# bryanboateng/animating-gaussian-splats

Measured on AMD Instinct MI355X. Metric: Msplats/sec fwd+bwd @1080p (1M gauss), higher is better.
Workload: dtype f32; 1 GPU; C3: 1000000 Gaussians, SH3, 1920x1080, 27-camera rig, 5 view(s)/GPU/step, fwd+bwd; gaussians=1000000, image=1920x1080, sh_degree=3, parallelism=camera-dp1, streams_per_gpu=3, submission=one host thread per stream, means2D=one fresh zero leaf per render (shared.py:38-41)

## Files before the change

animating-gaussian-splats_amd/csrc/gsr_forward.hip:

```cpp
#include "gsr_common.h"
#include "gsr_internal.h"

#include <algorithm>
#include <type_traits>

namespace gsr {

#ifdef GSR_TRACE
__device__ uint64_t *g_trace_fwd;
#ifdef GSR_TRACE
__device__ inline uint64_t trace_fwd_work(uint64_t batches, uint64_t walk, uint64_t evals) {
    return (batches << 40) | ((walk < 0xFFFFFull ? walk : 0xFFFFFull) << 20) | (evals < 0xFFFFFull ? evals : 0xFFFFFull);
}
#endif
__device__ uint64_t *g_trace_emit;
#define GSR_EMIT_STAMP(k)                                                                        \
    do {                                                                                         \
        if (g_trace_emit && threadIdx.x == 0)                                                    \
            g_trace_emit[4 * blockIdx.x + (k)] = __builtin_amdgcn_s_memrealtime();               \
    } while (0)
#else
#define GSR_EMIT_STAMP(k) do {} while (0)
#endif

// ... 225 lines not shown
            ranges[tl] = cnt ? make_uint2(ex, ex + cnt) : make_uint2(0, 0);
            tile_cursor[tl] = ex;
            seg_off[tl] = ex_s + is - sb;
            if (cnt > (uint32_t)kSortCap) {
                sort_lists[T - 1 - atomicAdd(&ctr[3], 1u)] = (uint32_t)tl;
                atomicMax(&ctr[4], cnt);
            } else if (cnt > (uint32_t)kFwdSortCap) {
                sort_lists[atomicAdd(&ctr[2], 1u)] = (uint32_t)tl;
            }
        }
    }
    drain_vmem();
    __builtin_amdgcn_fence(__ATOMIC_RELEASE, "workgroup");
    __syncthreads();
    if (threadIdx.x == 0) s_last = atomicAdd(&ctr[1], 1u) == gridDim.x - 1 ? 1u : 0u;
    __syncthreads();
    if (!s_last) return;
    const uint64_t fin = __hip_atomic_load(&look[gridDim.x - 1], __ATOMIC_RELAXED, __HIP_MEMORY_SCOPE_AGENT);
    const uint32_t K = (uint32_t)fin, n_seg = (uint32_t)(fin >> 32) & 0x3FFFFFFFu;
    {
        constexpr int kPer = kOrderBuckets / (kColW * kColG);
        uint32_t h[kPer], hs = 0;
#pragma unroll
        for (int i = 0; i < kPer; ++i) {
            h[i] = __hip_atomic_load(&lpt[threadIdx.x * kPer + i], __ATOMIC_RELAXED, __HIP_MEMORY_SCOPE_AGENT);
            hs += h[i];
        }
        uint32_t tt;
        uint32_t e = block_excl_scan_u32(hs, s_red, &tt);
#pragma unroll
        for (int i = 0; i < kPer; ++i) {
            lpt[threadIdx.x * kPer + i] = e;
            e += h[i];
        }
    }
    {
        const uint32_t bs = (int)threadIdx.x < NB ? block_sums[threadIdx.x] : 0u;
        uint32_t btot;
        const uint32_t bex = block_excl_scan_u32(bs, s_red, &btot);
        if ((int)threadIdx.x < NB) block_off[threadIdx.x] = bex;
    }
    if (threadIdx.x == 0) {
        const uint32_t n_mid = __hip_atomic_load(&ctr[2], __ATOMIC_RELAXED, __HIP_MEMORY_SCOPE_AGENT);
        const uint32_t n_long = __hip_atomic_load(&ctr[3], __ATOMIC_RELAXED, __HIP_MEMORY_SCOPE_AGENT);
        const uint32_t max_long = __hip_atomic_load(&ctr[4], __ATOMIC_RELAXED, __HIP_MEMORY_SCOPE_AGENT);
        seg_off[T] = n_seg;
        meta[0] = K;
        meta[1] = (cap && K <= cap && n_long == 0u) ? 1u : 0u;
        meta[2] = n_mid;
        if (host_words) {
            __hip_atomic_store(host_words + 1, n_mid, __ATOMIC_RELAXED, __HIP_MEMORY_SCOPE_SYSTEM);
            __hip_atomic_store(host_words + 2, n_long, __ATOMIC_RELAXED, __HIP_MEMORY_SCOPE_SYSTEM);
            __hip_atomic_store(host_words + 3, max_long, __ATOMIC_RELAXED, __HIP_MEMORY_SCOPE_SYSTEM);
            __hip_atomic_store(host_words, K, __ATOMIC_RELEASE, __HIP_MEMORY_SCOPE_SYSTEM);
        }
    }
}

__global__ __launch_bounds__(1024) void k_bin_scan(int T, int NB, const uint32_t *__restrict__ tile_count,
                                                   uint2 *__restrict__ ranges,
                                                   uint32_t *__restrict__ tile_cursor,
                                                   const uint32_t *__restrict__ block_sums,
                                                   uint32_t *__restrict__ block_off,
                                                   uint32_t *__restrict__ meta,
                                                   uint32_t *host_words,
                                                   uint32_t *__restrict__ tile_order,
                                                   uint32_t *__restrict__ sort_lists,
                                                   uint32_t *__restrict__ seg_off, uint32_t cap, int ks) {
    __shared__ uint32_t s_red[16];
    __shared__ uint32_t s_hist[kOrderBuckets];
    __shared__ uint32_t s_cls[3];
    if (threadIdx.x < 3) s_cls[threadIdx.x] = 0;
    uint32_t carry = 0;
    for (int base = 0; base < T; base += blockDim.x) {
        const int t = base + threadIdx.x;
        const uint32_t c = t < T ? tile_count[t] : 0;
        uint32_t tot;
        const uint32_t ex = block_excl_scan_u32(c, s_red, &tot) + carry;
        if (t < T) {
            ranges[t] = c ? make_uint2(ex, ex + c) : make_uint2(0, 0);
            tile_cursor[t] = ex;
        }
        carry += tot;
    }
    uint32_t carry3 = 0;
    for (int base = 0; base < T; base += blockDim.x) {
        const int t = base + threadIdx.x;
        const uint32_t nb = t < T ? seg_bounds(tile_count[t], ks) : 0;
        uint32_t tot;
        const uint32_t ex = block_excl_scan_u32(nb, s_red, &tot) + carry3;
        if (t < T) seg_off[t] = ex;
        carry3 += tot;
    }
    if (threadIdx.x == 0) seg_off[T] = carry3;
    uint32_t carry2 = 0;
    for (int base = 0; base < NB; base += blockDim.x) {
        const int b = base + threadIdx.x;
        const uint32_t c = b < NB ? block_sums[b] : 0;
        uint32_t tot;
        const uint32_t ex = block_excl_scan_u32(c, s_red, &tot) + carry2;
        if (b < NB) block_off[b] = ex;
        carry2 += tot;
    }
    __syncthreads();
    for (int t = threadIdx.x; t < T; t += blockDim.x) {
        const uint32_t n = tile_count[t];
        if (n == 0) continue;
        if (n > (uint32_t)kSortCap) {
            sort_lists[T - 1 - atomicAdd(&s_cls[1], 1u)] = (uint32_t)t;
            atomicMax(&s_cls[2], n);
        } else if (n > (uint32_t)kFwdSortCap) {
            sort_lists[atomicAdd(&s_cls[0], 1u)] = (uint32_t)t;
        }
    }
    lds_barrier();
    if (threadIdx.x == 0) {
        meta[0] = carry;
        meta[1] = (cap && carry <= cap && s_cls[1] == 0u) ? 1u : 0u;
        meta[2] = s_cls[0];
        if (host_words) {
            for (int c = 0; c < 3; ++c)
                __hip_atomic_store(host_words + 1 + c, s_cls[c], __ATOMIC_RELAXED, __HIP_MEMORY_SCOPE_SYSTEM);
            __hip_atomic_store(host_words, carry, __ATOMIC_RELEASE, __HIP_MEMORY_SCOPE_SYSTEM);
        }
    }
    lpt_order(T, [&](int t) { return tile_count[t]; }, tile_order, s_hist, s_red);
}

template <bool USE_LDS>
__global__ __launch_bounds__(kBinThreads) void k_bin_emit(int P, int CH, int T, int gx,
                                                  const uint2 *__restrict__ rects,
                                                  const uint32_t *__restrict__ tiles,
                                                  const float *__restrict__ depth,
                                                  const uint32_t *__restrict__ block_off,
                                                  uint32_t *__restrict__ tile_cursor,
                                                  uint32_t *__restrict__ goff,
                                                  uint4 *__restrict__ pairs, uint32_t K,
                                                  const uint32_t *__restrict__ chunk_off,
                                                  const uint32_t *__restrict__ spec_ok,
                                                  const uint32_t *__restrict__ tile_count,
                                                  const uint32_t *__restrict__ tile_rank,
                                                  const uint32_t *__restrict__ lpt_off,
                                                  uint32_t *__restrict__ tile_order) {
    extern __shared__ __attribute__((aligned(16))) uint32_t s_cur[];
    __shared__ uint32_t s_red[16];
    if (spec_ok && *spec_ok == 0u) return;
    const int b = blockIdx.x;
    const int g0 = b * CH, g1 = min(P, g0 + CH);
    if (tile_rank) {
        const int per = div_up(T, (int)gridDim.x), t1 = min(T, (b + 1) * per);
        for (int t = b * per + (int)threadIdx.x; t < t1; t += blockDim.x)
            tile_order[lpt_off[lpt_bucket(tile_count[t])] + tile_rank[t]] = (uint32_t)t;
    }
    GSR_EMIT_STAMP(0);
    if (USE_LDS) {
        const uint32_t *row = chunk_off + (size_t)b * T;
        for (int t = threadIdx.x; t < T; t += blockDim.x) s_cur[t] = tile_cursor[t] + row[t];
        __syncthreads();
        GSR_EMIT_STAMP(1);
        GSR_EMIT_STAMP(2);
    }
    uint32_t carry = block_off[b];
    for (int base = g0; base < g1; base += blockDim.x) {
        const int g = base + threadIdx.x;
        const uint32_t n = g < g1 ? tiles[g] : 0;
        uint32_t tot;
        const uint32_t ex = block_excl_scan_u32(n, s_red, &tot) + carry;
        carry += tot;
        if (g < g1) {
            goff[g] = ex;
            if (n) {
                const uint2 r = rects[g];
                const int x0 = r.x & 0xFFFF, y0 = r.x >> 16, x1 = r.y & 0xFFFF, y1 = r.y >> 16;
                const uint32_t dbits = __float_as_uint(depth[g]);
                uint32_t e = ex;
                for (int y = y0; y < y1; ++y)
                    for (int x = x0; x < x1; ++x, ++e) {
                        const int t = y * gx + x;
                        const uint32_t pos = USE_LDS ? atomicAdd(&s_cur[t], 1u) : atomicAdd(&tile_cursor[t], 1u);
                        pairs[pos] = make_uint4((uint32_t)g, dbits, e, 0u);
                    }
            }
        }
    }
    if (b == gridDim.x - 1 && threadIdx.x == 0) goff[P] = spec_ok ? spec_ok[-1] : K;
#ifdef GSR_TRACE
    __syncthreads();
    GSR_EMIT_STAMP(3);
#endif
}


template <int D>
__device__ inline uint32_t lane_xor(uint32_t x) {
    if constexpr (D == 1) return (uint32_t)__builtin_amdgcn_mov_dpp((int)x, 0xB1, 0xF, 0xF, false);
    else if constexpr (D == 2) return (uint32_t)__builtin_amdgcn_mov_dpp((int)x, 0x4E, 0xF, 0xF, false);
    else if constexpr (D == 4) {
        const int m = __builtin_amdgcn_mov_dpp((int)x, 0x141, 0xF, 0xF, false);
        return (uint32_t)__builtin_amdgcn_mov_dpp(m, 0x1B, 0xF, 0xF, false);
    } else if constexpr (D == 8) return (uint32_t)__builtin_amdgcn_mov_dpp((int)x, 0x128, 0xF, 0xF, false);
    else if constexpr (D == 16) {
        auto r = __builtin_amdgcn_permlane16_swap(x, x, false, false);
        return (threadIdx.x & 16) ? r[0] : r[1];
    } else {
        auto r = __builtin_amdgcn_permlane32_swap(x, x, false, false);
        return (threadIdx.x & 32) ? r[0] : r[1];
    }
}

template <int R, int D>
__device__ inline void bitonic_xlane(uint64_t (&k)[R], uint32_t (&v)[R], bool take_min) {
#pragma unroll
    for (int r = 0; r < R; ++r) {
        const uint32_t plo = lane_xor<D>((uint32_t)k[r]), phi = lane_xor<D>((uint32_t)(k[r] >> 32));
        const uint32_t pv = lane_xor<D>(v[r]);
        const uint64_t pk = ((uint64_t)phi << 32) | plo;
        const bool mine = (k[r] < pk) == take_min;
        k[r] = mine ? k[r] : pk;
        v[r] = mine ? v[r] : pv;
    }
}

template <int R, int J>
__device__ inline void wave_merge_stages(uint64_t (&k)[R], uint32_t (&v)[R], int lane, uint32_t gbase, uint32_t KK) {
    if constexpr (J > 0) {
        if constexpr (J < R) {
#pragma unroll
            for (int r = 0; r < R; ++r) {
                if (r & J) continue;
                const int r2 = r | J;
                const bool asc = ((gbase + lane * R + r) & KK) == 0;
                if ((k[r] > k[r2]) == asc) {
                    const uint64_t t = k[r]; k[r] = k[r2]; k[r2] = t;
                    const uint32_t u = v[r]; v[r] = v[r2]; v[r2] = u;
                }
            }
        } else {
            constexpr int D = J / R;
            const bool asc = ((gbase + lane * R) & KK) == 0;
            const bool take_min = ((lane & D) == 0) == asc;
            bitonic_xlane<R, D>(k, v, take_min);
        }
        wave_merge_stages<R, J / 2>(k, v, lane, gbase, KK);
    }
}

template <int R, int KK>
__device__ inline void wave_sort_stages(uint64_t (&k)[R], uint32_t (&v)[R], int lane, uint32_t gbase) {
    if constexpr (KK <= 64 * R) {
        wave_merge_stages<R, KK / 2>(k, v, lane, gbase, KK);
        wave_sort_stages<R, 2 * KK>(k, v, lane, gbase);
    }
}

__device__ inline uint32_t sort_slot(uint32_t i) { return i + (i >> 4); }
constexpr int sort_slots(int n) { return n + n / 16; }

template <int R>
__device__ inline void block_xchg_stage(uint64_t (&k)[R], uint32_t (&v)[R], uint32_t ibase, int kk, int j,
                                        uint64_t *s_key, uint32_t *s_val) {
    const uint32_t sb = sort_slot(ibase), qb = sort_slot(ibase ^ (uint32_t)j);
#pragma unroll
    for (int r = 0; r < R; ++r) { s_key[sb + r] = k[r]; s_val[sb + r] = v[r]; }
    __syncthreads();
#pragma unroll
    for (int r = 0; r < R; ++r) {
        const uint32_t i = ibase + r;
        const uint64_t pk = s_key[qb + r];
        const uint32_t pv = s_val[qb + r];
        const bool take_min = ((i & j) == 0) == ((i & kk) == 0);
        const bool mine = (k[r] < pk) == take_min;
        k[r] = mine ? k[r] : pk;
        v[r] = mine ? v[r] : pv;
    }
    __syncthreads();
}

template <int R, int NW>
__device__ inline void block_sort_tile(int n, uint32_t start, const uint4 *__restrict__ pairs, uint64_t *s_key,
                                       uint32_t *s_val) {
    constexpr int SEG = 64 * R;
    const int lane = threadIdx.x & 63, w = threadIdx.x >> 6;
    const uint32_t gbase = (uint32_t)(w * SEG), ibase = gbase + lane * R;
    uint64_t k[R];
    uint32_t v[R];
#pragma unroll
    for (int r = 0; r < R; ++r) {
        const int i = (int)ibase + r;
        const uint4 q = i < n ? pairs[start + i] : make_uint4(~0u, ~0u, 0u, 0u);
        k[r] = pair_key(q);
        v[r] = q.z;
    }
    wave_sort_stages<R, 2>(k, v, lane, gbase);
    for (uint32_t kk = 2 * SEG; kk <= (uint32_t)(NW * SEG); kk <<= 1) {
        for (uint32_t j = kk >> 1; j >= (uint32_t)SEG; j >>= 1) block_xchg_stage<R>(k, v, ibase, kk, j, s_key, s_val);
        wave_merge_stages<R, SEG / 2>(k, v, lane, gbase, kk);
    }
    const uint32_t sb = sort_slot(ibase);
#pragma unroll
    for (int r = 0; r < R; ++r) { s_key[sb + r] = k[r]; s_val[sb + r] = v[r]; }
    __syncthreads();
}

__global__ __launch_bounds__(512) void k_tile_sort(int gx, const uint32_t *__restrict__ tiles,
                                                    const uint2 *__restrict__ ranges,
                                                    uint4 *__restrict__ pairs,
                                                    uint32_t *__restrict__ point_list,
                                                    uint32_t *__restrict__ slot_emit, uint32_t nlist,
                                                    const uint32_t *__restrict__ spec_ok) {
    __shared__ uint64_t s_keys[sort_slots(kSortCap)];
    __shared__ uint32_t s_vals[sort_slots(kSortCap)];
    if (spec_ok) {
        if (*spec_ok == 0u) return;
        nlist = spec_ok[1];
    }
    static_assert(kSortCap == 8 * 64 * 8, "k_tile_sort: 8 waves x 64 lanes x 8 keys");
    for (uint32_t li = blockIdx.x; li < nlist; li += gridDim.x) {
        const int tile = (int)tiles[li];
        const uint2 rg = ranges[tile];
        const int n = (int)(rg.y - rg.x);
        if (n <= 4 * 64 * 8) block_sort_tile<4, 8>(n, rg.x, pairs, s_keys, s_vals);
        else block_sort_tile<8, 8>(n, rg.x, pairs, s_keys, s_vals);
        for (int i = threadIdx.x; i < n; i += blockDim.x) {
            const uint32_t sl = sort_slot((uint32_t)i);
            point_list[rg.x + i] = (uint32_t)s_keys[sl];
            slot_emit[rg.x + i] = s_vals[sl];
        }
        __syncthreads();
    }
}

__device__ inline uint4 key_record(uint64_t k, uint32_t emit) {
    return make_uint4((uint32_t)k, (uint32_t)(k >> 32), emit, 0u);
}

__global__ __launch_bounds__(512) void k_chunk_sort(int T, const uint32_t *__restrict__ lists,
                                                     const uint2 *__restrict__ ranges, uint4 *__restrict__ pairs) {
    __shared__ uint64_t s_keys[sort_slots(kSortCap)];
    __shared__ uint32_t s_vals[sort_slots(kSortCap)];
    const int tile = (int)lists[T - 1 - (int)blockIdx.y];
    const uint2 rg = ranges[tile];
    const int n = (int)(rg.y - rg.x);
    const int c0 = (int)blockIdx.x * kSortCap;
    if (c0 >= n) return;
    const int m = min(kSortCap, n - c0);
    block_sort_tile<8, 8>(m, rg.x + c0, pairs, s_keys, s_vals);
    for (int i = threadIdx.x; i < m; i += blockDim.x) {
        const uint32_t sl = sort_slot((uint32_t)i);
        pairs[rg.x + c0 + i] = key_record(s_keys[sl], s_vals[sl]);
    }
}

__device__ inline uint32_t merge_split(const uint4 *__restrict__ a, uint32_t la, const uint4 *__restrict__ b,
                                       uint32_t lb, uint32_t d) {
    const int lane = threadIdx.x & 63;
    uint32_t lo = d > lb ? d - lb : 0u, hi = min(d, la);
    while (lo < hi) {
        const uint32_t span = hi - lo, step = (span + 63) / 64;
        const uint32_t x = lo + (uint32_t)lane * step;
        const bool p = x < hi && pair_key(a[x]) < pair_key(b[d - 1 - x]);
        const uint32_t c = (uint32_t)__popcll(__ballot(p));
        const uint32_t nlo = c ? lo + (c - 1) * step + 1 : lo;
        const uint32_t nhi = min(hi, lo + c * step);
        lo = nlo;
        hi = max(nlo, nhi);
    }
    return lo;
}

__global__ __launch_bounds__(512) void k_merge_pass(int T, const uint32_t *__restrict__ lists,
                                                     const uint2 *__restrict__ ranges, uint32_t L,
                                                     const uint4 *__restrict__ src, uint4 *__restrict__ dst,
                                                     int final_pass, uint32_t *__restrict__ point_list,
                                                     uint32_t *__restrict__ slot_emit) {
    __shared__ uint64_t s_ka[kSortCap], s_kb[kSortCap];
    __shared__ uint32_t s_va[kSortCap], s_vb[kSortCap];
    __shared__ uint32_t s_split[2];
    const int tile = (int)lists[T - 1 - (int)blockIdx.y];
    const uint2 rg = ranges[tile];
    const uint32_t n = rg.y - rg.x;
    const uint32_t o0 = blockIdx.x * (uint32_t)kSortCap;
    if (o0 >= n) return;
    const uint32_t pb = o0 / (2 * L) * (2 * L);
    const uint32_t la = min(L, n - pb), lb = n - pb > L ? min(L, n - pb - L) : 0u;
    const uint4 *a = src + rg.x + pb, *b = a + la;
    const uint32_t d0 = o0 - pb, d1 = min(d0 + (uint32_t)kSortCap, la + lb);
    const int wv = threadIdx.x >> 6;
    if (wv < 2) {
        const uint32_t sp = merge_split(a, la, b, lb, wv == 0 ? d0 : d1);
        if ((threadIdx.x & 63) == 0) s_split[wv] = sp;
    }
    __syncthreads();
    const uint32_t i0 = s_split[0], i1 = s_split[1], j0 = d0 - i0, j1 = d1 - i1;
    const uint32_t na = i1 - i0, nb = j1 - j0;
    for (uint32_t i = threadIdx.x; i < na; i += blockDim.x) { const uint4 q = a[i0 + i]; s_ka[i] = pair_key(q); s_va[i] = q.z; }
    for (uint32_t i = threadIdx.x; i < nb; i += blockDim.x) { const uint4 q = b[j0 + i]; s_kb[i] = pair_key(q); s_vb[i] = q.z; }
    __syncthreads();
    constexpr uint32_t kPer = kSortCap / 512;
    const uint32_t dl = threadIdx.x * kPer;
    if (dl >= na + nb) return;
    uint32_t lo = dl > nb ? dl - nb : 0u, hi = min(dl, na);
    while (lo < hi) {
        const uint32_t mid = (lo + hi) >> 1;
        if (s_ka[mid] < s_kb[dl - 1 - mid]) lo = mid + 1; else hi = mid;
    }
    uint32_t ia = lo, ib = dl - lo;
    const uint32_t e = min(dl + kPer, na + nb);
    for (uint32_t o = dl; o < e; ++o) {
        const bool take_a = ib >= nb || (ia < na && s_ka[ia] < s_kb[ib]);
        const uint64_t k = take_a ? s_ka[ia] : s_kb[ib];
        const uint32_t v = take_a ? s_va[ia] : s_vb[ib];
        ia += take_a; ib += !take_a;
        const size_t slot = (size_t)rg.x + pb + d0 + o;
        if (final_pass) { point_list[slot] = (uint32_t)k; slot_emit[slot] = v; }
        else dst[slot] = key_record(k, v);
    }
}

__device__ inline void gate_wait(const uint32_t *gate, uint32_t seq, uint32_t *err, uint64_t timeout) {
    const uint64_t t0 = __builtin_amdgcn_s_memrealtime();
    while ((int32_t)(__hip_atomic_load(gate, __ATOMIC_ACQUIRE, __HIP_MEMORY_SCOPE_SYSTEM) - seq) < 0) {
        __builtin_amdgcn_s_sleep(100);
        if (__builtin_amdgcn_s_memrealtime() - t0 > timeout) {
            if (threadIdx.x == 0 &&
                (int32_t)(__hip_atomic_load(gate, __ATOMIC_ACQUIRE, __HIP_MEMORY_SCOPE_SYSTEM) - seq) < 0)
                __hip_atomic_store(err, seq, __ATOMIC_RELAXED, __HIP_MEMORY_SCOPE_SYSTEM);
            return;
        }
    }
}

#ifndef GSR_TSAT_THREADS
#define GSR_TSAT_THREADS 64
#endif
constexpr int kTSatThreads = GSR_TSAT_THREADS;
__device__ inline bool tsat_flagged(float T, uint32_t last) { return T < kTSat * (1.0f + t_window(last)); }
struct TSatRec { float4 r0, r1, r3; };
__device__ inline TSatRec tsat_load(const float4 *__restrict__ rec, uint32_t g, bool v) {
    TSatRec t;
    const float4 z = make_float4(0.f, 0.f, 0.f, 0.f);
    const float4 *r = rec + (size_t)kRecF4 * g;
    t.r0 = v ? r[0] : z; t.r1 = v ? r[1] : z; t.r3 = v ? r[3] : z;
    return t;
}
__device__ inline void tsat_chain(int nf, const uint32_t *__restrict__ plist, float pfx, float pfy,
                                  const float4 *__restrict__ rec, uint32_t *s_rc, float *s_q, float *s_a,
                                  uint32_t *s_pos, float &T, uint32_t &nex, float4 &E) {
    constexpr int NT = kTSatThreads, NW = NT / 64;
    const int t = threadIdx.x, lane = t & 63, wv = t >> 6;
    float Tc = 0.f;
    bool stopped = false;
    uint32_t g_next = t < nf ? plist[t] : 0u;
    TSatRec cur = tsat_load(rec, g_next, t < nf);
    g_next = NT + t < nf ? plist[NT + t] : 0u;
    for (int base = 0; base < nf; base += NT) {
        const int e = base + t;
        const TSatRec r = cur;
        cur = tsat_load(rec, g_next, e + NT < nf);
        g_next = e + 2 * NT < nf ? plist[e + 2 * NT] : 0u;
        bool take = false;
        float al = 0.f;
        if (e < nf) {
            const Blend eb = blend_eval<true>(r.r0, r.r1, pfx, pfy);
            if (eb.p2 <= 0.0f && eb.alpha >= kNearLo) {
                const ExactBlend x = exact_blend(r.r0.x, r.r0.y, r.r3, r.r1.y, pfx, pfy);
                take = eb.alpha >= kNearHi || (x.power <= 0.0f && x.alpha >= 1.0f / 255.0f);
                al = x.alpha;
            }
        }
        const uint64_t m = __ballot(take);
        if (lane == 0) s_rc[wv] = (uint32_t)__builtin_popcountll(m);
        __syncthreads();
        uint32_t off = 0, nc = 0;
#pragma unroll
        for (int w = 0; w < NW; ++w) {
            off += w < wv ? s_rc[w] : 0u;
            nc += s_rc[w];
        }
        if (take) {
            const uint32_t rk = off + __builtin_amdgcn_mbcnt_hi((uint32_t)(m >> 32), __builtin_amdgcn_mbcnt_lo((uint32_t)m, 0u));
            s_q[rk] = 1.0f - al;
            s_a[rk] = al;
            s_pos[rk] = (uint32_t)e;
        }
        if (t < 4) s_q[nc + t] = 1.0f;
        __syncthreads();
        if (wv == 0) {
            const float4 *q4 = reinterpret_cast<const float4 *>(s_q);
            for (uint32_t k = 0; k < nc; k += 4) {
                uint32_t j = 0;
                const uint32_t v = min(4u, nc - k);
                if (!stopped) {
                    const float4 q = q4[k >> 2];
                    const float t1 = T * q.x, t2 = t1 * q.y, t3 = t2 * q.z, t4 = t3 * q.w;
                    if (t4 >= kTSat) {
                        T = t4;
                        nex = s_pos[k + v - 1] + 1u;
                        continue;
                    }
                    const float tv[4] = {t1, t2, t3, t4};
                    while (tv[j] >= kTSat) ++j;
                    if (j > 0) {
                        T = tv[j - 1];
                        nex = s_pos[k + j - 1] + 1u;
                    }
                    stopped = true;
                    Tc = T;
                }
                for (; j < v; ++j) {
                    const float a = s_a[k + j];
                    const float4 c = rec[(size_t)kRecF4 * plist[s_pos[k + j]] + 2];
                    const float w = a * Tc;
                    E.x += c.x * w; E.y += c.y * w; E.z += c.z * w; E.w += c.w * w;
                    Tc = Tc * (1.0f - a);
                }
            }
        }
        __syncthreads();
    }
}
__device__ inline void tsat_store(int px, int py, int W, int H, int n, float4 pe, float dfast, float T, uint32_t nex,
                                  float4 E, const float *__restrict__ bg, float *__restrict__ out_color,
                                  float *__restrict__ out_depth, float4 *__restrict__ pix_end,
                                  uint32_t *__restrict__ n_contrib, size_t sb, float4 *__restrict__ seg_state, int ks,
                                  uint32_t *s_nex) {
    const int t = threadIdx.x;
    const int pid = py * W + px;
    const float4 fin = make_float4(pe.x - E.x, pe.y - E.y, pe.z - E.z, T);
    if (t == 0) {
        pix_end[pid] = fin;
        n_contrib[pid] = nex;
        out_color[pid] = fin.x + T * bg[0];
        out_color[H * W + pid] = fin.y + T * bg[1];
        out_color[2 * H * W + pid] = fin.z + T * bg[2];
        out_depth[pid] = dfast - E.w;
    }
    const uint32_t b0 = (nex + (1u << ks) - 1u) >> ks;
    const int lx = px % kTileW, ly = py % kTileH;
    const int bslot = 64 * (ly >> 2) + 16 * (ly & 3) + lx;
    const uint32_t nb = n > 0 ? (uint32_t)(n - 1) >> ks : 0u;
    for (uint32_t q = max(b0, 1u) + (uint32_t)t; q <= nb; q += kTSatThreads)
        seg_state[(sb + q - 1u) * kTilePix + bslot] = fin;
    (void)s_nex;
}
#define GSR_FWD_ATTR __attribute__((amdgpu_waves_per_eu(8, 8)))
template <bool EXACT>
__global__ __launch_bounds__(256) GSR_FWD_ATTR void k_render_fwd(
    int W, int H, int gx, int T, const uint32_t *__restrict__ tile_order, const uint2 *__restrict__ ranges,
    const uint4 *__restrict__ pairs,
    uint32_t *__restrict__ point_list, uint32_t *__restrict__ slot_emit, const float4 *__restrict__ rec,
    const float *__restrict__ bg, float *__restrict__ out_color, float *__restrict__ out_depth,
    float4 *__restrict__ pix_end, uint32_t *__restrict__ n_contrib, uint32_t *__restrict__ tile_maxc,
    const uint32_t *__restrict__ seg_off, float4 *__restrict__ seg_state, const uint32_t *__restrict__ spec_ok,
    int ks, const uint32_t *gate, uint32_t gate_seq, uint32_t *gate_err, uint64_t gate_timeout,
    uint32_t *__restrict__ tile_flag, float4 *__restrict__ near_rec, uint32_t *__restrict__ tsat_n,
    uint32_t *__restrict__ tsat_list, uint32_t tsat_cap) {
    __shared__ uint64_t s_key[sort_slots(kFwdSortCap > 0 ? kFwdSortCap : 1)];
    __shared__ union {
        uint32_t val[sort_slots(kFwdSortCap > 0 ? kFwdSortCap : 1)];
        struct {
            float4 rec[3][66];
            uint32_t q[64];
        } st;
    } s_u;
    __shared__ uint32_t s_live;
    __shared__ uint32_t s_near;
#ifdef GSR_TRACE
    const uint64_t t_start = __builtin_amdgcn_s_memrealtime();
#endif
    if (spec_ok && *spec_ok == 0u) {
        if (gate && blockIdx.x == 0 && threadIdx.x < 64) gate_wait(gate, gate_seq, gate_err, gate_timeout);
        return;
    }
    const int tile = (int)tile_order[blockIdx.x];
    const uint2 rg = ranges[tile];
    const int n = (int)(rg.y - rg.x);
    const bool sorted_here = n <= kFwdSortCap;
    if (threadIdx.x == 0) s_near = 0;
    if (n > 0 && sorted_here) {
        if (n <= 256) block_sort_tile<1, 4>(n, rg.x, pairs, s_key, s_u.val);
        else if (n <= 512) block_sort_tile<2, 4>(n, rg.x, pairs, s_key, s_u.val);
        else block_sort_tile<4, 4>(n, rg.x, pairs, s_key, s_u.val);
        for (int i = threadIdx.x; i < n; i += 256) {
            const uint32_t sl = sort_slot((uint32_t)i);
            point_list[rg.x + i] = (uint32_t)s_key[sl];
            slot_emit[rg.x + i] = s_u.val[sl];
        }
    }
    const int wv = threadIdx.x >> 6, lane = threadIdx.x & 63;
    const int tx = tile % gx, ty = tile / gx;
    const int lx = 8 * (wv & 1) + (lane & 7), ly = 8 * (wv >> 1) + (lane >> 3);
    const int px = tx * kTileW + lx;
    const int py = ty * kTileH + ly;
    const float pfx = (float)px, pfy = (float)py;
    const int bslot = 64 * (ly >> 2) + 16 * (ly & 3) + lx;
    const int se = threadIdx.x >> 2, sq = threadIdx.x & 3;
    const float qx0 = (float)(tx * kTileW + 8 * (sq & 1)), qy0 = (float)(ty * kTileH + 8 * (sq >> 1));
    constexpr int kQW = 8, kQH = 8;
    const bool inside = px < W && py < H;
    constexpr float kThrDone = 2.0f;
    constexpr float kThrLive = EXACT ? kNearLo : 1.0f / 255.0f;
    float thr = inside ? kThrLive : kThrDone;
    const uint32_t pix_key = (uint32_t)(16 * ly + lx);
    if (threadIdx.x == 0) s_live = 0;
    __syncthreads();
#ifdef GSR_TRACE
    const uint64_t tr_sorted = __builtin_amdgcn_s_memrealtime();
#endif
    if (__ballot(thr < kThrDone) && lane == 0) atomicOr(&s_live, 1u << wv);
    float Tt = 1.0f;
    f2v C01 = f2(0.f, 0.f), C2D = f2(0.f, 0.f);
    uint32_t last = 0;
    float4 pa = make_float4(0.f, 0.f, 0.f, 0.f), pb = pa, pr = pa;
    bool pv = false;
#define FETCH_BATCH(bse)                                                                           \
    do {                                                                                           \
        const int idx_ = (bse) + se;                                                               \
        pv = idx_ < n;                                                                             \
        if (pv) {                                                                                  \
            const uint32_t g_ = sorted_here ? (uint32_t)s_key[sort_slot(idx_)] : point_list[rg.x + idx_]; \
            const float4 *r_ = rec + (size_t)kRecF4 * g_;                                          \
            pa = r_[0];                                                                            \
            pb = r_[1];                                                                            \
            pr = r_[sq < 3 ? sq : 2];                                                              \
        }                                                                                          \
    } while (0)
    FETCH_BATCH(0);
#ifdef GSR_TRACE
    uint64_t tr_batches = 0, tr_walk = 0, tr_entries = 0;
#endif
    for (int base = 0; base < n; base += 64) {
        lds_barrier();
        const uint32_t live = s_live;
        if (!live) break;
        if (base > 0 && (base & ((1 << ks) - 1)) == 0) {
            const size_t b = (size_t)seg_off[tile] + ((uint32_t)base >> ks) - 1u;
            seg_state[b * kTilePix + bslot] = make_float4(C01.x, C01.y, C2D.x, Tt);
        }
        bool hit = false, opaque = false;
        {
            const float4 a = pa, b = pb;
            opaque = pv && b.y > 0.99f;
            if (pv) {
                if (sq < 3) s_u.st.rec[sq][se] = pr;
                hit = ((live >> sq) & 1u) &&
                      !tile_cull(a.x, a.y, -2.f * a.z, -a.w, -2.f * b.x, b.y, b.w, qx0, qy0, qx0 + (kQW - 1), qy0 + (kQH - 1));
            }
            FETCH_BATCH(base + 64);
        }
        uint32_t bits = hit ? (1u << sq) : 0u;
        bits |= (uint32_t)__builtin_amdgcn_mov_dpp((int)bits, 0xB1, 0xF, 0xF, false);
        bits |= (uint32_t)__builtin_amdgcn_mov_dpp((int)bits, 0x4E, 0xF, 0xF, false);
        if (sq == 0) s_u.st.q[se] = bits | ((bits && opaque) ? 16u : 0u);
        __syncthreads();
        const uint32_t qw = s_u.st.q[lane];
        uint64_t m = __ballot((qw >> wv) & 1u);
        if (!((live >> wv) & 1u)) m = 0;
        const bool clamp = __builtin_amdgcn_ballot_w64((qw & 16u) != 0u) != 0;
        const float t_stop = EXACT ? kTSat * (1.0f - t_window((uint32_t)base + 64u)) : kTSat;
        auto take = [&](const Blend &e, bool ok, float4 b, float4 c, int j) {
            const float test_T = fmaf(-e.alpha, Tt, Tt);
            const bool use = ok && test_T >= t_stop;
            thr = (ok && !use) ? kThrDone : thr;
            if (use) {
                const float w = e.alpha * Tt;
                C01 = fma2(f2(c.x, c.y), f2(w, w), C01);
                C2D = fma2(f2(c.z, c.w), f2(w, w), C2D);
                Tt = test_T;
                last = (uint32_t)(base + j + 1);
            }
        };
        auto walk = [&](auto clamp_c) {
            constexpr bool CL = decltype(clamp_c)::value;
            while (m) {
                const int j = __builtin_ctzll(m);
                m &= ~(1ull << j);
                const float4 a = s_u.st.rec[0][j], b = s_u.st.rec[1][j], c = s_u.st.rec[2][j];
                Blend e = blend_eval<CL>(a, b, pfx, pfy);
                bool ok = e.p2 <= 0.0f && e.alpha >= thr;
                if constexpr (EXACT) {
                    const bool nr = ok && e.alpha < kNearHi;
                    if (nr) {
                        const int idx = base + j;
                        const uint32_t g = sorted_here ? (uint32_t)s_key[sort_slot(idx)] : point_list[rg.x + idx];
                        const ExactBlend x = exact_blend(a.x, a.y, rec[(size_t)kRecF4 * g + 3], b.y, pfx, pfy);
                        e.p2 = x.power; e.G = x.G; e.alpha = x.alpha;
                        ok = x.power <= 0.0f && x.alpha >= 1.0f / 255.0f;
                        const uint32_t slot = atomicAdd(&s_near, 1u);
                        if (slot < kNearCap)
                            near_rec[(size_t)kNearCap * tile + slot] =
                                make_float4(__uint_as_float(((uint32_t)idx << 8) | pix_key), x.power, x.G, x.alpha);
                    }
                }
                take(e, ok, b, c, j);
            }
        };
#ifdef GSR_TRACE
        const uint64_t tr_w0 = __builtin_amdgcn_s_memrealtime();
        tr_batches += 1;
        tr_entries += (uint64_t)__builtin_popcountll(m);
#endif
        if (clamp) walk(std::true_type{});
        else walk(std::false_type{});
#ifdef GSR_TRACE
        tr_walk += __builtin_amdgcn_s_memrealtime() - tr_w0;
#endif
        if (((live >> wv) & 1u) && !__ballot(thr < kThrDone) && lane == 0) atomicAnd(&s_live, ~(1u << wv));
    }
    if (EXACT && inside && tsat_flagged(Tt, last)) {
        const uint32_t slot = atomicAdd(tsat_n, 1u);
        if (slot < tsat_cap) {
            uint4 *r = reinterpret_cast<uint4 *>(tsat_list) + 2 * (size_t)slot;
            r[0] = make_uint4((uint32_t)(py * W + px), rg.x, (uint32_t)n, last);
            r[1] = make_uint4(__float_as_uint(C01.x), __float_as_uint(C01.y), __float_as_uint(C2D.x), __float_as_uint(C2D.y));
        }
    }
    if (inside) {
        const int pid = py * W + px;
        pix_end[pid] = make_float4(C01.x, C01.y, C2D.x, Tt);
        n_contrib[pid] = last;
        out_color[pid] = C01.x + Tt * bg[0];
        out_color[H * W + pid] = C01.y + Tt * bg[1];
        out_color[2 * H * W + pid] = C2D.x + Tt * bg[2];
        out_depth[pid] = C2D.y;
    }
    uint32_t mx = last;
#pragma unroll
    for (int d = 16; d > 0; d >>= 1) mx = max(mx, (uint32_t)__shfl_xor((int)mx, d, 64));
    __syncthreads();
    if (threadIdx.x < 4) s_u.st.q[threadIdx.x] = 0;
    __syncthreads();
    if ((lane & 31) == 0) atomicMax(&s_u.st.q[2 * (wv >> 1) + (lane >> 5)], mx);
    lds_barrier();
    if (threadIdx.x < 4) tile_maxc[4 * tile + threadIdx.x] = s_u.st.q[threadIdx.x];
    if (threadIdx.x == 0) tile_flag[tile] = EXACT ? s_near : 0u;
#ifdef GSR_TRACE
    trace_wave(g_trace_fwd, 4 * blockIdx.x + wv, t_start, trace_fwd_work(tr_batches, tr_walk, tr_entries));
    if (g_trace_fwd && lane == 0)
        g_trace_fwd[4 * (4 * blockIdx.x + wv) + 2] |= (tr_sorted - t_start) << 40;
#endif
}

#ifndef GSR_TSAT_BLOCKS
#define GSR_TSAT_BLOCKS 4096
#endif
constexpr int kTSatBlocks = GSR_TSAT_BLOCKS;
__global__ __launch_bounds__(kTSatThreads) void k_render_tsat(
    int W, int H, const uint32_t *__restrict__ point_list, const float4 *__restrict__ rec,
    const float *__restrict__ bg, float *__restrict__ out_color, float *__restrict__ out_depth,
    float4 *__restrict__ pix_end, uint32_t *__restrict__ n_contrib, const uint32_t *__restrict__ seg_off,
    float4 *__restrict__ seg_state, const uint32_t *__restrict__ tsat_n, const uint32_t *__restrict__ tsat_list,
    uint32_t tsat_cap, const uint32_t *__restrict__ spec_ok, int ks, int gx, const uint2 *__restrict__ ranges) {
    constexpr int NT = kTSatThreads;
    __shared__ float4 s_buf[(3 * NT + 4 + 3) / 4];
    __shared__ uint32_t s_rc[4];
    if (spec_ok && *spec_ok == 0u) return;
    const uint32_t flagged = *tsat_n;
    const uint32_t cnt = flagged > tsat_cap ? 0u : flagged;
#ifdef GSR_TRACE
    const uint64_t tr_b = __builtin_amdgcn_s_memrealtime();
#endif
    float *s_q = reinterpret_cast<float *>(s_buf), *s_a = s_q + NT + 4;
    uint32_t *s_pos = reinterpret_cast<uint32_t *>(s_a + NT);
    for (uint32_t i = blockIdx.x; i < cnt; i += gridDim.x) {
#ifdef GSR_TRACE
        const uint64_t tr_i = __builtin_amdgcn_s_memrealtime();
#endif
        const uint4 *rp = reinterpret_cast<const uint4 *>(tsat_list) + 2 * (size_t)i;
        const uint4 r0 = rp[0], r1 = rp[1];
        const uint32_t pid = r0.x, start = r0.y;
        const int n = (int)r0.z, nf = (int)r0.w;
        const int px = (int)(pid % (uint32_t)W), py = (int)(pid / (uint32_t)W);
        const int tile = (py / kTileH) * gx + px / kTileW;
        float T = 1.0f;
        uint32_t nex = 0;
        float4 E = make_float4(0.f, 0.f, 0.f, 0.f);
        tsat_chain(nf, point_list + start, (float)px, (float)py, rec, s_rc, s_q, s_a, s_pos, T, nex, E);
#ifdef GSR_TRACE
        const uint64_t tr_c = __builtin_amdgcn_s_memrealtime();
#endif
        if (threadIdx.x == 0) {
            s_rc[0] = nex;
            s_rc[1] = __float_as_uint(T);
            s_q[0] = E.x; s_q[1] = E.y; s_q[2] = E.z; s_q[3] = E.w;
        }
        __syncthreads();
        tsat_store(px, py, W, H, n,
                   make_float4(__uint_as_float(r1.x), __uint_as_float(r1.y), __uint_as_float(r1.z), 0.f),
                   __uint_as_float(r1.w), __uint_as_float(s_rc[1]), s_rc[0],
                   make_float4(s_q[0], s_q[1], s_q[2], s_q[3]), bg, out_color, out_depth, pix_end, n_contrib,
                   seg_off[tile], seg_state, ks, nullptr);
        __syncthreads();
#ifdef GSR_TRACE
        const uint32_t ntile = (uint32_t)gx * (uint32_t)((H + kTileH - 1) / kTileH);
        if (g_trace_fwd && threadIdx.x == 0 && i < 4u * ntile) {
            uint64_t *o = g_trace_fwd + 16 * (size_t)ntile + 4 * (size_t)i;
            o[0] = tr_i;
            o[1] = __builtin_amdgcn_s_memrealtime();
            o[2] = (uint64_t)(uint32_t)nf | ((uint64_t)(uint32_t)n << 32);
            o[3] = (tr_c - tr_i) | ((tr_i - tr_b) << 32);
        }
#endif
    }
    if (__builtin_expect(flagged > tsat_cap, 0)) {
        const uint32_t npix = (uint32_t)W * (uint32_t)H;
        for (uint32_t base = blockIdx.x * 64u; base < npix; base += gridDim.x * 64u) {
            const uint32_t p = base + (threadIdx.x & 63u);
            uint64_t fm = __ballot(p < npix && tsat_flagged(pix_end[p].w, n_contrib[p]));
            __syncthreads();
            while (fm) {
                const uint32_t pid = base + (uint32_t)__builtin_ctzll(fm);
                fm &= fm - 1;
                const int px = (int)(pid % (uint32_t)W), py = (int)(pid / (uint32_t)W);
                const int tile = (py / kTileH) * gx + px / kTileW;
                const uint2 rg = ranges[tile];
                const float4 pe = pix_end[pid];
                const int nf = (int)n_contrib[pid];
                const float dfast = out_depth[pid];
                float T = 1.0f;
                uint32_t nex = 0;
                float4 E = make_float4(0.f, 0.f, 0.f, 0.f);
                tsat_chain(nf, point_list + rg.x, (float)px, (float)py, rec, s_rc, s_q, s_a, s_pos, T, nex, E);
                if (threadIdx.x == 0) {
                    s_rc[0] = nex;
                    s_rc[1] = __float_as_uint(T);
                    s_q[0] = E.x; s_q[1] = E.y; s_q[2] = E.z; s_q[3] = E.w;
                }
                __syncthreads();
                tsat_store(px, py, W, H, (int)(rg.y - rg.x), make_float4(pe.x, pe.y, pe.z, 0.f), dfast,
                           __uint_as_float(s_rc[1]), s_rc[0], make_float4(s_q[0], s_q[1], s_q[2], s_q[3]), bg,
                           out_color, out_depth, pix_end, n_contrib, seg_off[tile], seg_state, ks, nullptr);
                __syncthreads();
            }
        }
    }
}

__global__ void k_zero_f32(float *p, size_t n) {
    const size_t i = (size_t)blockIdx.x * blockDim.x + threadIdx.x;
    if (i < n) p[i] = 0.f;
}

__global__ void k_mark_visible(int P, const float *__restrict__ means3D,
                               const float *__restrict__ viewmatrix, uint8_t *__restrict__ present) {
    const int i = blockIdx.x * blockDim.x + threadIdx.x;
    if (i >= P) return;
    float vm[16];
#pragma unroll
    for (int k = 0; k < 16; ++k) vm[k] = viewmatrix[k];
    const float3 pv = xform4x3(make_float3(means3D[3 * i], means3D[3 * i + 1], means3D[3 * i + 2]), vm);
    present[i] = !(pv.z <= 0.2f);
}

template <int MC>
static void preprocess_mc(const FwdArgs &a, hipStream_t s) {
    k_preprocess<MC><<<div_up(a.v.P, kShBlock), kShBlock, sizeof(float) * kShBlock * (MC ? sh_row_stride(MC) : 0), s>>>(
        a.v.P, a.v.D, a.v.M, a.v.means3D, a.v.scales, a.v.scale_modifier, a.v.rotations, a.v.opacities, a.v.shs,
        a.v.colors_precomp, a.v.cov3D_precomp, a.v.viewmatrix, a.v.projmatrix, a.v.campos, a.v.W, a.v.H, a.v.tan_fovx,
        a.v.tan_fovy, a.v.focal_x, a.v.focal_y, a.v.gx, a.v.gy, a.radii, a.depth, a.rec, a.rect, a.tiles, a.v.act, a.v.cs,
        a.tile_count, a.v.gx * a.v.gy, a.clampm);
}

hipError_t launch_preprocess(const FwdArgs &a, hipStream_t s) {
    if (a.v.P == 0) return hipSuccess;
    const int mc = a.v.shs ? a.v.M : 0;
    switch (mc) {
        case 16: preprocess_mc<16>(a, s); break;
        case 9: preprocess_mc<9>(a, s); break;
        case 4: preprocess_mc<4>(a, s); break;
        case 1: preprocess_mc<1>(a, s); break;
        default: preprocess_mc<0>(a, s); break;
    }
    return hipGetLastError();
}

hipError_t launch_bin_count(const FwdArgs &a, hipStream_t s) {
    const BinGrid bg(a.v.P);
    const int T = a.v.gx * a.v.gy;
    if (bg.NB == 0) return hipSuccess;
    if (T <= kMaxLdsTiles)
        k_bin_count<true><<<bg.NB, kBinThreads, sizeof(uint32_t) * T, s>>>(a.v.P, bg.CH, T, a.v.gx, a.rect, a.tiles, a.tile_count, a.block_sums, a.chunk_off, a.items_ws, a.scan_ws);
    else
        k_bin_count<false><<<bg.NB, kBinThreads, 0, s>>>(a.v.P, bg.CH, T, a.v.gx, a.rect, a.tiles, a.tile_count, a.block_sums, nullptr, a.items_ws, nullptr);
    return hipGetLastError();
}

hipError_t launch_bin_scan(const FwdArgs &a, uint32_t *host_words, hipStream_t s) {
    const BinGrid bg(a.v.P);
    const int T = a.v.gx * a.v.gy;
    if (T <= kMaxLdsTiles && bg.NB > 0)
        k_bin_colscan<<<div_up(T, kColW), kColW * kColG, 0, s>>>(T, bg.NB, a.chunk_off, a.tile_count, a.ranges,
                                                                a.tile_cursor, a.seg_off, a.sort_lists, a.tile_rank,
                                                                a.scan_ws, a.block_sums, a.block_off, a.meta,
                                                                host_words, a.spec_cap, seg_log2(a.v.P));
    else
        k_bin_scan<<<1, 1024, 0, s>>>(T, bg.NB, a.tile_count, a.ranges, a.tile_cursor,
                                      a.block_sums, a.block_off, a.meta, host_words, a.tile_order_f,
                                      a.sort_lists, a.seg_off, a.spec_cap, seg_log2(a.v.P));
    return hipGetLastError();
}

hipError_t launch_bin_emit(const FwdArgs &a, int K, hipStream_t s) {
    const BinGrid bg(a.v.P);
    const int T = a.v.gx * a.v.gy;
    if (bg.NB == 0) return hipSuccess;
    if (T <= kMaxLdsTiles)
        k_bin_emit<true><<<bg.NB, kBinThreads, sizeof(uint32_t) * T, s>>>(a.v.P, bg.CH, T, a.v.gx, a.rect, a.tiles, a.depth, a.block_off, a.tile_cursor, a.goff, a.pairs, (uint32_t)K, a.chunk_off, a.spec_ok,
                                                                           a.tile_count, a.tile_rank, a.scan_ws + 2 * kScanBlocksMax + kScanCtr, a.tile_order_f);
    else
        k_bin_emit<false><<<bg.NB, kBinThreads, 0, s>>>(a.v.P, bg.CH, T, a.v.gx, a.rect, a.tiles, a.depth, a.block_off, a.tile_cursor, a.goff, a.pairs, (uint32_t)K, a.chunk_off, a.spec_ok,
                                                        nullptr, nullptr, nullptr, nullptr);
    return hipGetLastError();
}

hipError_t launch_tile_sort(const FwdArgs &a, uint32_t n_mid, uint32_t n_vlong, uint32_t max_n, uint4 *tmp,
                            hipStream_t s) {
    const int T = a.v.gx * a.v.gy;
    if (a.spec_ok) {
        const int nb = a.spec_sort_blocks ? (int)a.spec_sort_blocks : kSpecSortBlocks;
        k_tile_sort<<<std::min(T, nb), 512, 0, s>>>(a.v.gx, a.sort_lists, a.ranges, a.pairs, a.point_list,
                                                                 a.slot_emit, 0u, a.spec_ok);
        return hipGetLastError();
    }
    if (n_mid) k_tile_sort<<<n_mid, 512, 0, s>>>(a.v.gx, a.sort_lists, a.ranges, a.pairs, a.point_list, a.slot_emit,
                                                 n_mid, nullptr);
    if (n_vlong) {
        const dim3 grid((unsigned)div_up((int)max_n, kSortCap), n_vlong);
        k_chunk_sort<<<grid, 512, 0, s>>>(T, a.sort_lists, a.ranges, a.pairs);
        const uint4 *src = a.pairs;
        uint4 *dst = tmp;
        for (uint32_t L = kSortCap; L < max_n; L *= 2) {
            const int final_pass = 2 * (size_t)L >= max_n;
            k_merge_pass<<<grid, 512, 0, s>>>(T, a.sort_lists, a.ranges, L, src, dst, final_pass, a.point_list,
                                              a.slot_emit);
            const uint4 *t = dst;
            dst = const_cast<uint4 *>(src);
            src = t;
        }
    }
    return hipGetLastError();
}

hipError_t launch_render_fwd(const FwdArgs &a, hipStream_t s) {
    const int T = a.v.gx * a.v.gy;
    auto k = a.exact ? k_render_fwd<true> : k_render_fwd<false>;
    k<<<T, 256, 0, s>>>(a.v.W, a.v.H, a.v.gx, T, a.tile_order_f, a.ranges, a.pairs,
                        a.point_list, a.slot_emit, a.rec, a.v.bg, a.out_color, a.out_depth, a.pix_end, a.n_contrib,
                        a.tile_maxc, a.seg_off, a.seg_state, a.spec_ok, seg_log2(a.v.P), a.gate, a.gate_seq,
                        a.gate_err, a.gate_timeout, a.tile_flag, a.near_rec, a.items_ws + kTSatCtr, a.tsat_list,
                        tsat_capacity(a.v.W * a.v.H));
    if (a.exact)
        k_render_tsat<<<kTSatBlocks, kTSatThreads, 0, s>>>(a.v.W, a.v.H, a.point_list, a.rec, a.v.bg, a.out_color, a.out_depth,
                                                 a.pix_end, a.n_contrib, a.seg_off, a.seg_state, a.items_ws + kTSatCtr,
                                                 a.tsat_list, tsat_capacity(a.v.W * a.v.H), a.spec_ok, seg_log2(a.v.P),
                                                 a.v.gx, a.ranges);
    return hipGetLastError();
}

hipError_t launch_zero(float *p, size_t n, hipStream_t s) {
    if (n == 0) return hipSuccess;
    k_zero_f32<<<(unsigned)((n + 255) / 256), 256, 0, s>>>(p, n);
    return hipGetLastError();
}

hipError_t launch_mark_visible(int P, const float *means3D, const float *viewmatrix, uint8_t *present,
                               hipStream_t s) {
    if (P == 0) return hipSuccess;
    k_mark_visible<<<div_up(P, 256), 256, 0, s>>>(P, means3D, viewmatrix, present);
    return hipGetLastError();
}

}

#ifdef GSR_TRACE
extern "C" int gsr_debug_trace_fwd(void *buf) {
    return hipMemcpyToSymbol(HIP_SYMBOL(gsr::g_trace_fwd), &buf, sizeof(buf)) == hipSuccess ? 0 : 2;
}
extern "C" int gsr_debug_trace_emit(void *buf) {
    return hipMemcpyToSymbol(HIP_SYMBOL(gsr::g_trace_emit), &buf, sizeof(buf)) == hipSuccess ? 0 : 2;
}
#endif
```

Before: 1398 Msplats/s.

## Replace per-tile bitonic sort with depth-bucketed counting sort and fallback

Adds a block-level bucket sort for per-tile depth keys. It scans the depth range, scatters keys into linearly spaced buckets with shared-memory atomics, prefix-scans the counts, and ranks keys within each small bucket by direct comparison. If any bucket overflows its cap or depths are non-finite, it falls back to the existing bitonic sort. The aim is to replace the O(n log^2 n) bitonic network with near-linear work in both the forward render sort and the large-tile sort kernel. The cost is extra shared memory (which may reduce occupancy) and wasted work whenever the fallback triggers.

Result: no change. 1395 Msplats/s (-0.3%).

```diff
diff --git a/animating-gaussian-splats_amd/csrc/gsr_forward.hip b/animating-gaussian-splats_amd/csrc/gsr_forward.hip
--- a/animating-gaussian-splats_amd/csrc/gsr_forward.hip
+++ b/animating-gaussian-splats_amd/csrc/gsr_forward.hip
@@ -551,6 +551,150 @@
     __syncthreads();
 }
 
+#ifndef GSR_BUCKET_SORT
+#define GSR_BUCKET_SORT 1
+#endif
+#ifndef GSR_BUCKET_CAP
+#define GSR_BUCKET_CAP 16
+#endif
+constexpr int kBucketCap = GSR_BUCKET_CAP;
+#ifndef GSR_BUCKET_MIN
+#define GSR_BUCKET_MIN 129
+#endif
+constexpr int kBucketMin = GSR_BUCKET_MIN;
+
+__device__ inline uint32_t wave_min_u32(uint32_t x) {
+    x = min(x, lane_xor<1>(x)); x = min(x, lane_xor<2>(x)); x = min(x, lane_xor<4>(x));
+    x = min(x, lane_xor<8>(x)); x = min(x, lane_xor<16>(x)); x = min(x, lane_xor<32>(x));
+    return x;
+}
+__device__ inline uint32_t wave_max_u32(uint32_t x) {
+    x = max(x, lane_xor<1>(x)); x = max(x, lane_xor<2>(x)); x = max(x, lane_xor<4>(x));
+    x = max(x, lane_xor<8>(x)); x = max(x, lane_xor<16>(x)); x = max(x, lane_xor<32>(x));
+    return x;
+}
+
+template <int R, int NW, bool EARLY = false>
+__device__ inline bool block_bucket_sort_tile(int n, uint32_t start, const uint4 *__restrict__ pairs, uint64_t *s_key,
+                                              uint32_t *s_val, uint32_t *s_cnt, uint32_t *s_red) {
+    constexpr int NT = 64 * NW;
+    const int t = threadIdx.x, lane = t & 63, w = t >> 6;
+    const int rows = (n + NT - 1) / NT;
+    const int nb = rows * NT;
+    uint64_t k[R];
+    uint32_t v[R];
+    uint32_t dlo = ~0u, dhi = 0u;
+#pragma unroll
+    for (int r = 0; r < R; ++r) {
+        if (r >= rows) break;
+        const int i = t + NT * r;
+        s_cnt[i] = 0u;
+        const uint4 q = i < n ? pairs[start + i] : make_uint4(0u, 0u, 0u, 0u);
+        k[r] = pair_key(q);
+        v[r] = q.z;
+        if (i < n) { dlo = min(dlo, q.y); dhi = max(dhi, q.y); }
+    }
+    dlo = wave_min_u32(dlo);
+    dhi = wave_max_u32(dhi);
+    if (lane == 0) { s_red[w] = dlo; s_red[NW + w] = dhi; }
+    if (t == 0) s_red[2 * NW] = 0u;
+    __syncthreads();
+#pragma unroll
+    for (int x = 0; x < NW; ++x) { dlo = min(dlo, s_red[x]); dhi = max(dhi, s_red[NW + x]); }
+    if (dhi >= 0x7F800000u) return false;
+    const float dmin = __uint_as_float(dlo), dmax = __uint_as_float(dhi);
+    const float inv = dmax > dmin ? (float)nb / (dmax - dmin) : 0.0f;
+    const float bmax = (float)(nb - 1);
+    uint32_t bp[R];
+    bool over = false;
+#pragma unroll
+    for (int r = 0; r < R; ++r) {
+        if (r >= rows) break;
+        const int i = t + NT * r;
+        if (i < n) {
+            const uint32_t b = (uint32_t)(int)fminf((__uint_as_float((uint32_t)(k[r] >> 32)) - dmin) * inv, bmax);
+            const uint32_t place = atomicAdd(&s_cnt[b], 1u);
+            over |= place >= (uint32_t)kBucketCap;
+            bp[r] = b | (place << 16);
+        }
+        if (EARLY && r == 0 && rows > 1) {
+            if (__ballot(over) && lane == 0) s_red[2 * NW] = 1u;
+            __syncthreads();
+            if (s_red[2 * NW]) return false;
+        }
+    }
+    if (__ballot(over) && lane == 0) s_red[2 * NW] = 1u;
+    __syncthreads();
+    if (s_red[2 * NW]) return false;
+    uint32_t c[R], sum = 0u;
+#pragma unroll
+    for (int r = 0; r < R; ++r) {
+        if (r >= rows) break;
+        c[r] = s_cnt[t * rows + r];
+        sum += c[r];
+    }
+    uint32_t tot;
+    uint32_t ex = block_excl_scan_u32(sum, s_red, &tot);
+    (void)tot;
+#pragma unroll
+    for (int r = 0; r < R; ++r) {
+        if (r >= rows) break;
+        s_cnt[t * rows + r] = ex;
+        ex += c[r];
+    }
+    if (t == NT - 1) s_cnt[nb] = ex;
+    __syncthreads();
+    uint32_t bs[R], bn[R];
+#pragma unroll
+    for (int r = 0; r < R; ++r) {
+        if (r >= rows) break;
+        if (t + NT * r < n) {
+            const uint32_t b = bp[r] & 0xFFFFu;
+            bs[r] = s_cnt[b];
+            bn[r] = s_cnt[b + 1] - bs[r];
+            s_key[bs[r] + (bp[r] >> 16)] = k[r];
+        }
+    }
+    __syncthreads();
+#pragma unroll
+    for (int r = 0; r < R; ++r) {
+        if (r >= rows) break;
+        if (t + NT * r < n) {
+            uint32_t rank = 0u;
+            if (bn[r] > 1u)
+                for (uint32_t j = 0; j < bn[r]; j += 4) {
+                    const uint64_t *m = s_key + bs[r] + j;
+                    const uint64_t m0 = m[0], m1 = m[1], m2 = m[2], m3 = m[3];
+                    rank += (m0 < k[r] ? 1u : 0u) + (j + 1 < bn[r] && m1 < k[r] ? 1u : 0u) +
+                            (j + 2 < bn[r] && m2 < k[r] ? 1u : 0u) + (j + 3 < bn[r] && m3 < k[r] ? 1u : 0u);
+                }
+            bs[r] += rank;
+        }
+    }
+    __syncthreads();
+#pragma unroll
+    for (int r = 0; r < R; ++r) {
+        if (r >= rows) break;
+        if (t + NT * r < n) {
+            const uint32_t sl = sort_slot(bs[r]);
+            s_key[sl] = k[r];
+            s_val[sl] = v[r];
+        }
+    }
+    __syncthreads();
+    return true;
+}
+
+#ifdef GSR_TRACE
+__device__ uint32_t *g_trace_sort;
+#define GSR_SORT_COUNT(slot)                                                                     \
+    do {                                                                                         \
+        if (g_trace_sort && threadIdx.x == 0) atomicAdd(&g_trace_sort[slot], 1u);                \
+    } while (0)
+#else
+#define GSR_SORT_COUNT(slot) do {} while (0)
+#endif
+
 __global__ __launch_bounds__(512) void k_tile_sort(int gx, const uint32_t *__restrict__ tiles,
                                                     const uint2 *__restrict__ ranges,
                                                     uint4 *__restrict__ pairs,
@@ -559,6 +703,10 @@
                                                     const uint32_t *__restrict__ spec_ok) {
     __shared__ uint64_t s_keys[sort_slots(kSortCap)];
     __shared__ uint32_t s_vals[sort_slots(kSortCap)];
+#if GSR_BUCKET_SORT
+    __shared__ uint32_t s_cnt[kSortCap + 1];
+    __shared__ uint32_t s_red[2 * 8 + 1];
+#endif
     if (spec_ok) {
         if (*spec_ok == 0u) return;
         nlist = spec_ok[1];
@@ -568,8 +716,15 @@
         const int tile = (int)tiles[li];
         const uint2 rg = ranges[tile];
         const int n = (int)(rg.y - rg.x);
-        if (n <= 4 * 64 * 8) block_sort_tile<4, 8>(n, rg.x, pairs, s_keys, s_vals);
-        else block_sort_tile<8, 8>(n, rg.x, pairs, s_keys, s_vals);
+        bool done = false;
+#if GSR_BUCKET_SORT
+        done = block_bucket_sort_tile<8, 8, true>(n, rg.x, pairs, s_keys, s_vals, s_cnt, s_red);
+        GSR_SORT_COUNT(done ? 2 : 3);
+#endif
+        if (!done) {
+            if (n <= 4 * 64 * 8) block_sort_tile<4, 8>(n, rg.x, pairs, s_keys, s_vals);
+            else block_sort_tile<8, 8>(n, rg.x, pairs, s_keys, s_vals);
+        }
         for (int i = threadIdx.x; i < n; i += blockDim.x) {
             const uint32_t sl = sort_slot((uint32_t)i);
             point_list[rg.x + i] = (uint32_t)s_keys[sl];
@@ -793,6 +948,7 @@
     (void)s_nex;
 }
 #define GSR_FWD_ATTR __attribute__((amdgpu_waves_per_eu(8, 8)))
+[[maybe_unused]] constexpr int kFwdRows = kFwdSortCap > 0 ? (kFwdSortCap + 255) / 256 : 1;
 template <bool EXACT>
 __global__ __launch_bounds__(256) GSR_FWD_ATTR void k_render_fwd(
     int W, int H, int gx, int T, const uint32_t *__restrict__ tile_order, const uint2 *__restrict__ ranges,
@@ -812,6 +968,11 @@
             uint32_t q[64];
         } st;
     } s_u;
+#if GSR_BUCKET_SORT
+    __shared__ uint32_t s_cnt[256 * kFwdRows + 1];
+    static_assert(kFwdSortCap <= 0 || sort_slots(kFwdSortCap) >= kFwdSortCap + 3, "the rank loop reads 3 slots past a bucket");
+    __shared__ uint32_t s_red[2 * 4 + 1];
+#endif
     __shared__ uint32_t s_live;
     __shared__ uint32_t s_near;
 #ifdef GSR_TRACE
@@ -827,9 +988,18 @@
     const bool sorted_here = n <= kFwdSortCap;
     if (threadIdx.x == 0) s_near = 0;
     if (n > 0 && sorted_here) {
-        if (n <= 256) block_sort_tile<1, 4>(n, rg.x, pairs, s_key, s_u.val);
-        else if (n <= 512) block_sort_tile<2, 4>(n, rg.x, pairs, s_key, s_u.val);
-        else block_sort_tile<4, 4>(n, rg.x, pairs, s_key, s_u.val);
+        bool done = false;
+#if GSR_BUCKET_SORT
+        if (n >= kBucketMin) {
+            done = block_bucket_sort_tile<kFwdRows, 4>(n, rg.x, pairs, s_key, s_u.val, s_cnt, s_red);
+            GSR_SORT_COUNT(done ? 0 : 1);
+        }
+#endif
+        if (!done) {
+            if (n <= 256) block_sort_tile<1, 4>(n, rg.x, pairs, s_key, s_u.val);
+            else if (n <= 512) block_sort_tile<2, 4>(n, rg.x, pairs, s_key, s_u.val);
+            else block_sort_tile<4, 4>(n, rg.x, pairs, s_key, s_u.val);
+        }
         for (int i = threadIdx.x; i < n; i += 256) {
             const uint32_t sl = sort_slot((uint32_t)i);
             point_list[rg.x + i] = (uint32_t)s_key[sl];
@@ -1225,6 +1395,9 @@
 extern "C" int gsr_debug_trace_fwd(void *buf) {
     return hipMemcpyToSymbol(HIP_SYMBOL(gsr::g_trace_fwd), &buf, sizeof(buf)) == hipSuccess ? 0 : 2;
 }
+extern "C" int gsr_debug_trace_sort(void *buf) {
+    return hipMemcpyToSymbol(HIP_SYMBOL(gsr::g_trace_sort), &buf, sizeof(buf)) == hipSuccess ? 0 : 2;
+}
 extern "C" int gsr_debug_trace_emit(void *buf) {
     return hipMemcpyToSymbol(HIP_SYMBOL(gsr::g_trace_emit), &buf, sizeof(buf)) == hipSuccess ? 0 : 2;
 }
```
